# BiaPyX/BiaPy

Measured on AMD Instinct MI355X. Metric: voxels/sec 3D ResUNet 128^3 patch (train: fwd+bwd+AdamW; sub-records: infer, sliding), higher is better.
Workload: dtype f16 forward/activations + bf16 gradients (MFMA f16 / bf16, fp32 accumulate)

## Files before the change

### biapy_amd/_lib.py

```python
from __future__ import annotations

import ctypes as C
import os
from typing import Optional

import torch

_HERE = os.path.dirname(os.path.abspath(__file__))
LIB_PATH = os.environ.get("BPX_LIB_PATH") or os.path.join(_HERE, "libbiapy_amd.so")

F32, BF16, F16, U8, MIX16 = 0, 1, 2, 3, 4
U16 = 5
I32 = 6
ACT = {"none": 0, "linear": 0, "elu": 1, "relu": 2, "silu": 3, "leaky_relu": 4, "gelu": 5, "tanh": 6, "sigmoid": 7, "softplus": 8}
PK_K3, PK_K3_T, PK_K1, PK_DENSE, PK_DENSE_T, PK_CT, PK_CT_T, PK_CT4, PK_CT4_T = range(9)


class AxisGrid(C.Structure):
    _fields_ = [("n", C.c_int32), ("step", C.c_int32), ("last", C.c_int32), ("patch", C.c_int32), ("limit", C.c_int32)]


class Tensor(C.Structure):
    _fields_ = [("ptr", C.c_void_p), ("ld", C.c_int32), ("C", C.c_int32), ("cs", C.c_int64)]


NULL_T = Tensor(None, 0, 0, 0)

_vp, _i, _i64, _f = C.c_void_p, C.c_int, C.c_int64, C.c_float

_SIGS = {
    "bpx_version": ([], C.c_int),
    "bpx_last_error": ([], C.c_char_p),
    "bpx_selftest_layouts": ([_vp, _vp], _i),
    "bpx_debug_set_wgrad_tr": ([_i], _i),
    "bpx_debug_set_conv_ws": ([_i], _i),
    "bpx_debug_set_conv_stamps": ([_vp], _i),
    "bpx_debug_set_tiling_scalar": ([_i], _i),
    "bpx_debug_set_conv_occ": ([_i], _i),
    "bpx_debug_set_conv_zm": ([_i], _i),
    "bpx_debug_conv_zm_launches": ([], _i),
    "bpx_debug_conv_zm_occupancy": ([_i], _i),
    "bpx_crop3d_gather": ([_vp, _i, _i, _i, _i, _i, _i, _i, _i, _i, C.POINTER(AxisGrid), _i64, _i64, _vp, _vp], _i),
    "bpx_merge3d_blend": ([_vp, _i, _i, _i, _i, _i, _i, _i, _i, C.POINTER(AxisGrid), _vp, _vp, _vp, _i, _i, _i, _i, _i, _i, _i,
                           _vp, _vp, _i, _vp, _i, _vp], _i),
    "bpx_packed_weight_elems": ([_i, _i, _i, _i], _i64),
    "bpx_pack_weight": ([_i, _vp, _i, _i, _i, _vp, _vp], _i),
    "bpx_pack_weights_batched": ([_i, _i, _vp, _vp], _i),
    "bpx_adam_step": ([_i, _vp, _vp, C.c_double, C.c_double, C.c_double, C.c_double, C.c_double, _i, _vp], _i),
    "bpx_grad_norm_workspace": ([_i, _vp], _i64),
    "bpx_grad_norm": ([_i, _vp, C.c_double, _vp, _i64, _vp, _vp], _i),
    "bpx_adam_step_dev": ([_i, _vp, _vp, C.c_double, _vp, C.c_double, C.c_double, C.c_double, C.c_double, _i, _vp, _vp], _i),
    "bpx_sgd_step": ([_i, _vp, _vp, C.c_double, _vp, C.c_double, C.c_double, C.c_double, _i, _vp, _vp], _i),
    "bpx_aug_draw": ([_vp, _i, _i, _i, _i, _vp, _vp, _vp], _i),
    "bpx_aug_mean_blocks": ([_i64], _i),
    "bpx_aug_mean": ([_vp, _i, _i64, _vp, _vp, _vp], _i),
    "bpx_aug_apply": ([_vp, _vp, _i, _i, _i, _i, _i, _i, _i, _vp, C.c_uint64, _f, _i, _vp, _vp, _vp], _i),
    "bpx_warp_draw": ([_vp, _i, _i, _i, _vp, _vp, _vp], _i),
    "bpx_warp_apply": ([_vp, _vp, _i, _i, _i, _i, _i, _i, _i, _vp, _i, _f, _vp, _vp, _vp], _i),
    "bpx_patch_draw": ([_vp, _vp, _vp, _vp, _vp, _i64, _i, _vp, _vp, _vp], _i),
    "bpx_patch_gather": ([_vp, _vp, _i, _i, _i, _i, _i, _i, _i, _i, _vp, _i, _i, _f, _vp, _vp, _vp], _i),
    "bpx_label_workspace": ([_i, _i, _i], _i64),
    "bpx_label_u8": ([_vp, _i, _i, _i, _i, _vp, _vp, _vp, _i64, _vp], _i),
    "bpx_label_sizes": ([_vp, _i64, _i, _vp, _vp], _i),
    "bpx_label_filter": ([_vp, _i64, _i, _vp, _i, _i, _vp, _vp], _i),
    "bpx_debug_set_label_tiled": ([_i], _i),
    "bpx_edt_workspace": ([_i, _i, _i, _i], _i64),
    "bpx_edt": ([_vp, _i, _i, _i, _i, _i, C.POINTER(C.c_double), _i, _vp, _vp, _i64, _vp], _i),
    "bpx_watershed_workspace": ([_i, _i, _i], _i64),
    "bpx_watershed": ([_vp, _i, _vp, _vp, _i, _i, _i, _i, _vp, _vp, _vp, _i64, _vp], _i),
    "bpx_overlap_workspace": ([_i64], _i64),
    "bpx_label_overlap": ([_vp, _vp, _i64, _i64, _vp, _vp, _vp, _vp, _i64, _vp], _i),
    "bpx_debug_set_overlap_per_voxel": ([_i], _i),
    "bpx_region_props": ([_vp, _i, _i, _i, _i, _vp, _vp, _vp, _vp], _i),
    "bpx_debug_set_regionprops_local": ([_i], _i),
    "bpx_morph": ([_vp, _i, _i, _i, _i, _i, _i, _i, _i, _i, _vp, _vp], _i),
    "bpx_peaks_workspace": ([_i, _i, _i], _i64),
    "bpx_peak_local_max": ([_vp, _i, _i, _i, _i, _i, _i, _i, C.c_double, _i, _i, _i, _vp, _vp, _i, _vp, _vp, _i64, _vp], _i),
    "bpx_scan_blocks": ([_i64], _i),
    "bpx_select_workspace": ([], _i64),
    "bpx_select_kth_f32": ([_vp, _i64, _i64, _vp, _vp, _vp], _i),
    "bpx_minmax_f32": ([_vp, _i64, _vp, _vp], _i),
    "bpx_moment_f32": ([_vp, _i64, C.c_double, _i, _vp, _vp], _i),
    "bpx_histogram_f32": ([_vp, _i64, _f, _f, _i, _vp, _vp, _vp], _i),
    "bpx_threshold_u8": ([_vp, _i64, _f, _vp, _vp], _i),
    "bpx_clip_affine_f32": ([_vp, _i64, _f, _f, _f, _f, _vp, _vp], _i),
    "bpx_class_argmax": ([_vp, _i64, _i, _i, _vp, _vp], _i),
    "bpx_tta_orient": ([_vp, _i, _i, _i, _i, _vp, _vp, _vp, _vp], _i),
    "bpx_tta_accumulate": ([_vp, _i, _i, _i, _i, _vp, _vp, _i, _i, _i, _vp, _vp], _i),
    "bpx_chan_loss_blocks": ([_i64], _i),
    "bpx_chan_loss_sums": ([_vp, _vp, _i, _i, _i64, C.c_uint, _vp, _vp], _i),
    "bpx_chan_loss_bwd": ([_vp, _vp, _i, _i, _i64, C.c_uint, _vp, _vp, _vp], _i),
    "bpx_gate_mul_fwd": ([_i, _i64, Tensor, Tensor, Tensor, _vp], _i),
    "bpx_gate_mul_bwd": ([_i, _i64, Tensor, Tensor, Tensor, Tensor, _vp, _vp], _i),
    "bpx_seg_loss_blocks": ([_i64], _i),
    "bpx_seg_loss_sums": ([_vp, _vp, _i64, _vp, _vp], _i),
    "bpx_seg_loss_bwd": ([_vp, _vp, _i64, _vp, _vp, _vp], _i),
    "bpx_seg_loss_finish": ([_vp, _i, _i64, _f, _f, _f, _vp, _vp, _vp], _i),
    "bpx_seg_loss_bwd_fused": ([_vp, _vp, _i64, _vp, _vp, _f, _f, _f, _vp, _vp], _i),
    "bpx_softmax_ce_blocks": ([_i64], _i),
    "bpx_softmax_ce_row": ([], _i),
    "bpx_softmax_ce_sums": ([_vp, _vp, _i, _i, _i64, _i, _vp, _vp, _vp], _i),
    "bpx_softmax_ce_finish": ([_vp, _i, _i64, _vp, _vp, _vp], _i),
    "bpx_softmax_ce_bwd": ([_vp, _vp, _i, _i, _i64, _i, _vp, _vp, _vp, _vp, _vp], _i),
    "bpx_dice_blocks": ([_i64], _i),
    "bpx_dice_row": ([], _i),
    "bpx_dice_sums": ([_vp, _vp, _i, _i, _i64, _i, _i, _vp, _i, _vp, _vp], _i),
    "bpx_dice_finish": ([_vp, _i, _i, _i64, _i, _i, C.c_double, C.c_double, C.c_double, _vp, _vp, _vp, _vp], _i),
    "bpx_dice_bwd": ([_vp, _vp, _i, _i, _i64, _i, _i, _i, _vp, _vp, _vp, _vp, _vp], _i),
    "bpx_chan_loss_finish": ([_vp, _i, _i, _i64, _vp, _vp, _vp], _i),
    "bpx_chan_loss_bwd_fused": ([_vp, _vp, _i, _i, _i64, C.c_uint, _vp, _vp, _vp, _vp], _i),
    "bpx_conv3d_fwd": ([_i, _i, _i, _i, _i, Tensor, _vp, _i, _vp, _vp, Tensor, _vp, _vp, Tensor, _vp, _vp], _i),
    "bpx_conv3d_fwd_pool": ([_i, _i, _i, _i, _i, Tensor, _vp, _i, _vp, _vp, Tensor, _vp, _vp, Tensor, _vp, _i, Tensor, _vp, _vp], _i),
    "bpx_conv3d_fwd_pool_supported": ([_i, _i, _i, _i, _i, _i, _i, _i], _i),
    "bpx_conv3d_fwd_shuffle": ([_i, _i, _i, _i, _i, Tensor, _vp, _i, _vp, _vp, _i, Tensor, _vp], _i),
    "bpx_conv3d_stats_tiles": ([_i, _i, _i, _i, _i, _i], _i),
    "bpx_conv3d_dgrad": ([_i, _i, _i, _i, _i, Tensor, _vp, Tensor, _vp, _i, Tensor, _vp, _vp], _i),
    "bpx_conv3d_wgrad": ([_i, _i, _i, _i, _i, Tensor, _vp, _i, Tensor, _i, _vp, _vp, _vp, _i64, _vp], _i),
    "bpx_conv3d_wgrad_db2": ([_i, _i, _i, _i, _i, Tensor, _vp, _i, Tensor, _i, _vp, _vp, _vp, _vp, _i64, _vp], _i),
    "bpx_conv3d_wgrad_workspace": ([_i, _i, _i, _i, _i, _i, _i], _i64),
    "bpx_conv3d_bwd_fused_supported": ([_i, _i, _i, _i, _i, _i, _i], _i),
    "bpx_conv3d_bwd_fused_stats_tiles": ([_i, _i, _i, _i, _i, _i], _i),
    "bpx_conv3d_bwd_fused_workspace": ([_i, _i, _i, _i, _i, _i], _i64),
    "bpx_conv3d_bwd_fused": ([_i, _i, _i, _i, _i, Tensor, _vp, Tensor, _vp, _i, Tensor, _vp, _vp, _vp, _vp, _vp, _i64, _vp], _i),
    "bpx_debug_set_bwd_fused": ([_i], _i),
# ... 261 lines not shown
```

### biapy_amd/csrc/conv3d_zmarch.hip

```cpp
#include "conv3d_shared.h"

using namespace bpxconv;

namespace {

#ifndef BPX_ZM_IMG_EARLY
#define BPX_ZM_IMG_EARLY 1
#endif

#ifndef BPX_ZM_RH
#define BPX_ZM_RH 4
#endif
#ifndef BPX_ZM_SCK_AH
#define BPX_ZM_SCK_AH 2
#endif
#ifndef BPX_ZM_SCK_RH
#define BPX_ZM_SCK_RH 2
#endif
constexpr int zm_occ(int nch, bool sck = false) { return (nch == 1 && !sck) ? 3 : 2; }

template <int NCH, int ACTK, bool F16, bool SCK = false>
__global__ void __launch_bounds__(256, zm_occ(NCH, SCK)) conv3_zm_kernel(const Conv3Params p) {
  using T = typename std::conditional<F16, f16_t, uint16_t>::type;
  constexpr int TZ = 4, TY = 8, TX = 16, MS = 8, KPL = 8, VB = 32, HY = TY + 2, HX = TX + 2;
  constexpr int PLANE_B = HY * HX * VB;
  constexpr int PP = HY * HX * 2;
  constexpr int PL = PP - 256;
  static_assert(2 * PL <= 256, "a plane pair's left-over pieces fit one round");
  constexpr int STEPS = 14, QPAD = 56, HSTR = HX * VB;
  constexpr int RH = NCH != 1 ? MS : SCK ? BPX_ZM_SCK_RH : BPX_ZM_RH;
  constexpr int PLANES = NCH == 1 ? 6 : 2 + 4 * NCH;
  constexpr int RING_B = PLANES * PLANE_B;
  constexpr int WLDS_B = NCH == 1 ? STEPS * 1024 : 0;
  constexpr int RED_B = (NCH == 1 ? 2 : 1) * 4 * 16 * 2 * 4;
  constexpr int TAB_B = NCH * 16 * 8 + 128;
  constexpr int POOL_B = NCH == 1 ? 2 * (MS / 2) * 32 * 8 : 0;
  constexpr int WOFF = RING_B, ROFF = WOFF + WLDS_B, TOFF = ROFF + RED_B, POFF = TOFF + TAB_B;
  __shared__ __attribute__((aligned(16))) unsigned char smem[POFF + POOL_B];
  float* const red = reinterpret_cast<float*>(smem + ROFF);
  float* const tab = reinterpret_cast<float*>(smem + TOFF);

  const int tid = threadIdx.x, lane = tid & 63;
  const int wave = __builtin_amdgcn_readfirstlane(tid >> 6);
  const int j = lane & 15, g = lane >> 4;
  const int D = p.D, H = p.H, W = p.W;
  constexpr int Cout = 16;
  const int cg_off = (g & 1) * 16;
  const bool hi_tap = (g >> 1) != 0;
  const uint32_t hb = (uint32_t)(j * VB + cg_off);

#ifdef BPX_ZM_STAMPS
  long long* stamps = (p.stamps && tid == 0) ? p.stamps + (size_t)blockIdx.x * 16 : nullptr;
  int stamp_i = 0, it = 0;
#define ZM_STAMP() do { if (stamps && it == 4 && stamp_i < 15) stamps[stamp_i++] = (long long)__builtin_readcyclecounter(); } while (0)
#define ZM_STEP_DONE() ++it
#else
#define ZM_STAMP() do { } while (0)
#define ZM_STEP_DONE() do { } while (0)
#endif

  const int sub = tid & 1;
  const int hvA = tid >> 1, hyA = hvA / HX, hxA = hvA - hyA * HX;
  const int selL = tid / PL, idxL = 256 + (tid - selL * PL), hvL = idxL >> 1, hyL = hvL / HX, hxL = hvL - hyL * HX;
  const bool hasL = tid < 2 * PL;
  const uint32_t HWB = (uint32_t)(H * W * p.x_ld) * 2u;
  uint32_t relA = (uint32_t)((hyA * W + hxA) * p.x_ld + sub * KPL) * 2u;
  uint32_t relL = (uint32_t)((hyL * W + hxL) * p.x_ld + sub * KPL) * 2u + (hasL ? (uint32_t)selL * HWB : 0u);
  asm volatile("" : "+v"(relA), "+v"(relL));
  const uint32_t ldsA = (uint32_t)tid * 16u, ldsL = (uint32_t)idxL * 16u;
  const char* __restrict__ xin = reinterpret_cast<const char*>(p.x);
  const char* __restrict__ wp = reinterpret_cast<const char*>(p.wp);
  const uint32_t wlane = (uint32_t)((g * Cout + j) * KPL) * 2u;
  const uint32_t x_csb = (uint32_t)p.x_cs * 2u, sc_csb = (uint32_t)p.sc_cs * 2u;

  const bool rank1 = p.sc != nullptr && p.sc_C == 1;
  float* const ektab = tab + NCH * 16 * 2;
  if (tid < 16) {
    float a = 0.f;
    if (p.bias) a += p.bias[tid];
    if (p.sc && p.bias_sc) a += p.bias_sc[tid];
    ektab[tid] = a;
    ektab[16 + tid] = rank1 ? reinterpret_cast<const float*>(p.wsc)[tid] : 0.f;
  }
  if constexpr (NCH == 1) {
#pragma unroll
    for (int q = tid; q < STEPS * 64; q += 256)
      *reinterpret_cast<u32x4_t*>(smem + WOFF + q * 16) = *reinterpret_cast<const u32x4_t*>(wp + (uint32_t)q * 16u);
  }

  const int tilesZ = p.tilesZ, colsPerSample = p.tilesY * p.tilesX;
  const int xcd = blockIdx.x & 7, slot = blockIdx.x >> 3, spx = gridDim.x >> 3;
  const int T8 = p.tilesPerXcd;
  int L0 = xcd * T8 + (int)(((long long)slot * T8) / spx), L1 = xcd * T8 + (int)(((long long)(slot + 1) * T8) / spx);
  {
    const int cap = min((xcd + 1) * T8, p.totalTiles);
    L1 = min(L1, cap);
  }
  if (L0 >= L1) return;
  int col = L0 / tilesZ, tzi = L0 - col * tilesZ;

  int n = 0, y0 = 0, x0 = 0, tyi = 0, txi = 0;
// ... 586 lines not shown
      for (int k = 0; k < MS / 2; ++k) {
        u32x2_t pk[2];
#pragma unroll
        for (int h = 0; h < 2; ++h) {
          const int ms = 2 * k + h;
          const bool in = okzx && ms < yrem;
          float v[4];
#pragma unroll
          for (int r = 0; r < 4; ++r) {
            const float t = acc[ms][r] + addk[r] + img[ms] * w1k[r];
            v[r] = in ? t : 0.f;
            s1[r] += v[r];
            s2[r] += v[r] * v[r];
          }
          pk[h] = u32x2_t{pk16s<T>(v[0], v[1]), pk16s<T>(v[2], v[3])};
          __builtin_amdgcn_raw_buffer_store_b64(pk[h], rs_y, (int)(in ? yb0 + ms * yrow : 0xFFFFFFFFu), 0, 0);
        }
        if (p.pool != nullptr) {
          const u32x2_t a = pk[0], b = pk[1];
          m[k][0] = fmaxf(lo16<T>(a[0]), lo16<T>(b[0])); m[k][1] = fmaxf(hi16<T>(a[0]), hi16<T>(b[0]));
          m[k][2] = fmaxf(lo16<T>(a[1]), lo16<T>(b[1])); m[k][3] = fmaxf(hi16<T>(a[1]), hi16<T>(b[1]));
#pragma unroll
          for (int r = 0; r < 4; ++r)
            m[k][r] = fmaxf(m[k][r], __builtin_bit_cast(float, __builtin_amdgcn_update_dpp(0, __builtin_bit_cast(int, m[k][r]), 0xB1, 0xF, 0xF, true)));
        }
      }
      if (p.part != nullptr) {
        float* red = reinterpret_cast<float*>(smem + ROFF) + par * 256;
#pragma unroll
        for (int r = 0; r < 4; ++r) {
          const float a = row16_sum(s1[r]), b = row16_sum(s2[r]);
          if (j == 0) *reinterpret_cast<f32x2_t*>(&red[(wave * 16 + g * 4 + r) * 2]) = f32x2_t{a, b};
        }
      }
      if (pool2 && (wave & 1)) {
        u32x2_t* ex = reinterpret_cast<u32x2_t*>(smem + POFF);
#pragma unroll
        for (int k = 0; k < MS / 2; ++k) ex[((wave >> 1) * (MS / 2) + k) * 32 + (lane >> 1)] = u32x2_t{pk16<T>(m[k][0], m[k][1]), pk16<T>(m[k][2], m[k][3])};
      }
    }
    if (pool2) __syncthreads();
    if (p.pool != nullptr) {
      float q1[4] = {0.f, 0.f, 0.f, 0.f}, q2[4] = {0.f, 0.f, 0.f, 0.f};
      if (pool2 && !(wave & 1)) {
        const u32x2_t* ex = reinterpret_cast<const u32x2_t*>(smem + POFF);
#pragma unroll
        for (int k = 0; k < MS / 2; ++k) {
          const u32x2_t o = ex[((wave >> 1) * (MS / 2) + k) * 32 + (lane >> 1)];
          m[k][0] = fmaxf(m[k][0], lo16<T>(o[0])); m[k][1] = fmaxf(m[k][1], hi16<T>(o[0]));
          m[k][2] = fmaxf(m[k][2], lo16<T>(o[1])); m[k][3] = fmaxf(m[k][3], hi16<T>(o[1]));
        }
      }
      if ((p.pool_sz == 1 || !(wave & 1)) && !(j & 1) && z0 + wave < D && x0 + j < W) {
        const int Dp = D / p.pool_sz, Hp = H >> 1, Wp = W >> 1;
        const int pz_ = (z0 + wave) / p.pool_sz, px = (x0 + j) >> 1;
        char* __restrict__ pout = reinterpret_cast<char*>(p.pool);
#pragma unroll
        for (int k = 0; k < MS / 2; ++k) {
          if (y0 + 2 * k < H) {
            const int py = (y0 >> 1) + k;
            *reinterpret_cast<u32x2_t*>(pout + (uint32_t)((((n * Dp + pz_) * Hp + py) * Wp + px) * p.pool_ld + g * 4) * 2u) =
                u32x2_t{pk16<T>(m[k][0], m[k][1]), pk16<T>(m[k][2], m[k][3])};
#pragma unroll
            for (int r = 0; r < 4; ++r) { q1[r] += m[k][r]; q2[r] += m[k][r] * m[k][r]; }
          }
        }
      }
      if (p.pool_part != nullptr) {
        float* red = reinterpret_cast<float*>(smem + ROFF) + par * 256 + 128;
#pragma unroll
        for (int r = 0; r < 4; ++r) {
          const float a = row16_sum(q1[r]), b = row16_sum(q2[r]);
          if (j == 0) *reinterpret_cast<f32x2_t*>(&red[(wave * 16 + g * 4 + r) * 2]) = f32x2_t{a, b};
        }
      }
    }
    __syncthreads();
    ZS_STEP_END()
  }
#undef ZS_STEP_BEGIN
#undef ZS_STEP_END
}

int g_zm_mode = -1;
int g_zm_wgs = 0;
int g_zm_launches = 0;

}

extern "C" int bpx_debug_conv_zm_launches(void) { return g_zm_launches; }
extern "C" int bpx_debug_conv_zm_occupancy(int nch) {
  int n = 0;
  hipError_t e = nch == 0   ? hipOccupancyMaxActiveBlocksPerMultiprocessor(&n, conv3_zs_kernel<1, true>, 512, 0)
                 : nch == 1 ? hipOccupancyMaxActiveBlocksPerMultiprocessor(&n, conv3_zm_kernel<1, 1, true>, 256, 0)
                            : hipOccupancyMaxActiveBlocksPerMultiprocessor(&n, conv3_zm_kernel<3, 1, true>, 256, 0);
  return e == hipSuccess ? n : -1;
}
extern "C" int bpx_debug_set_conv_zm(int mode) {
  g_zm_mode = mode < 0 ? -1 : (mode & 0xFF);
  g_zm_wgs = mode < 0 ? 0 : (mode >> 8);
  return 0;
}

namespace bpxconv {

static int zm_cu_count() {
  static int n = 0;
  if (n == 0) {
    int dev = 0, v = 0;
    n = (hipGetDevice(&dev) == hipSuccess && hipDeviceGetAttribute(&v, hipDeviceAttributeMultiprocessorCount, dev) == hipSuccess && v > 0) ? v : 256;
  }
  return n;
}

int launch_conv3_zm(const Conv3Params& p0, const TileCfg& c, hipStream_t s) {
  int mode = g_zm_mode, wgs = g_zm_wgs;
  if (mode < 0) {
    static const char* e = getenv("BPX_CONV_ZM");
    const int v = e ? atoi(e) : 1;
    mode = v & 0xFF; wgs = v >> 8;
  }
  const bool no_zs = (mode & 4) != 0;
  mode &= 3;
  if (mode == 0) return 1;
  if (!(c.tz == 4 && c.ty == 8 && c.tx == 16 && c.ns == 1) || p0.Cout != 16 || p0.ps > 1) return 1;
  if (!(p0.Cin == 16 || p0.Cin == 48)) return 1;
  if (p0.pool != nullptr && p0.Cin != 16) return 1;
  {
    static const char* e = getenv("BPX_CONV_ZM_MASK");
    static const int mask = e ? atoi(e) : 7;
    const int kind = p0.Cin == 48 ? 4 : (p0.sc != nullptr && p0.sc_C >= 16) ? 2 : 1;
    if (!(mask & kind)) return 1;
  }
  Conv3Params p = p0;
  p.tilesZ = cdiv(p.D, c.tz);
  p.tilesY = cdiv(p.H, c.ty);
  p.tilesX = cdiv(p.W, c.tx);
  p.tilesPerSample = p.tilesZ * p.tilesY * p.tilesX;
  p.totalTiles = p.N * p.tilesPerSample;
  p.tilesPerXcd = cdiv(p.totalTiles, 8);
  p.stamps = g_conv_stamps;
  p.dbg = 0;
  const int nch = p.Cin / 16;
  const bool sck = p.sc != nullptr && p.sc_C >= 16;
  {
    static const char* e = getenv("BPX_CONV_ZS");
    static const int zs = e ? atoi(e) : 1;
    if (zs && !no_zs && nch == 1 && !sck) {
      int gz = std::max(8, (zm_cu_count() * 2) & ~7);
      if (wgs > 0) gz = std::max(8, std::min(gz, wgs & ~7));
      gz = std::min(gz, 8 * p.tilesPerXcd);
      if (mode == 1 && (p.totalTiles < 4 * gz || p.tilesZ < 4)) return 1;
      const bool elu_ = p.act == BPX_ACT_ELU;
      ++g_zm_launches;
      dim3 gridz((unsigned)gz, 1);
      if (p.f16) { if (elu_) conv3_zs_kernel<1, true><<<gridz, 512, 0, s>>>(p); else conv3_zs_kernel<0, true><<<gridz, 512, 0, s>>>(p); }
      else { if (elu_) conv3_zs_kernel<1, false><<<gridz, 512, 0, s>>>(p); else conv3_zs_kernel<0, false><<<gridz, 512, 0, s>>>(p); }
      return 0;
    }
  }
  if (sck && (p.sc_C > 48 || nch != 1)) return 1;
  const int occ = zm_occ(nch, sck);
  int gx = std::max(8, (zm_cu_count() * occ) & ~7);
  if (wgs > 0) gx = std::max(8, std::min(gx, wgs & ~7));
  gx = std::min(gx, 8 * p.tilesPerXcd);
  if (mode == 1 && (p.totalTiles < 4 * gx || p.tilesZ < 4)) return 1;
  const bool elu = p.act == BPX_ACT_ELU;
  dim3 grid((unsigned)gx, 1);
#define Z(NCH, SCK)                                                                    \
  if (nch == NCH && sck == SCK) {                                                      \
    ++g_zm_launches;                                                                   \
    if (p.f16) {                                                                       \
      if (elu) conv3_zm_kernel<NCH, 1, true, SCK><<<grid, 256, 0, s>>>(p);             \
      else conv3_zm_kernel<NCH, 0, true, SCK><<<grid, 256, 0, s>>>(p);                 \
    } else {                                                                           \
      if (elu) conv3_zm_kernel<NCH, 1, false, SCK><<<grid, 256, 0, s>>>(p);            \
      else conv3_zm_kernel<NCH, 0, false, SCK><<<grid, 256, 0, s>>>(p);                \
    }                                                                                  \
    return 0;                                                                          \
  }
  Z(1, false) Z(1, true) Z(3, false)
#undef Z
  return 1;
}

}
```

### include/biapy_amd.h

```cpp
#ifndef BIAPY_AMD_H
#define BIAPY_AMD_H

#include <stdint.h>

#ifdef __cplusplus
extern "C" {
#endif

typedef void* bpx_stream_t;

enum bpx_dtype { BPX_F32 = 0, BPX_BF16 = 1, BPX_F16 = 2, BPX_U8 = 3,
                 BPX_MIX16 = 4,
                 BPX_U16 = 5,
                 BPX_I32 = 6 };
enum bpx_act { BPX_ACT_NONE = 0, BPX_ACT_ELU = 1, BPX_ACT_RELU = 2, BPX_ACT_SILU = 3, BPX_ACT_LEAKY_RELU = 4, BPX_ACT_GELU = 5, BPX_ACT_TANH = 6,
               BPX_ACT_SIGMOID = 7, BPX_ACT_SOFTPLUS = 8, BPX_ACT_LAST = 8 };
enum bpx_pad_mode { BPX_PAD_REFLECT = 0, BPX_PAD_ZEROS = 1 };

int bpx_version(void);
const char* bpx_last_error(void);
int bpx_selftest_layouts(float* out_d , bpx_stream_t stream);
int bpx_debug_set_wgrad_tr(int use_tr);
int bpx_debug_set_conv_stamps(void* stamps_d);
int bpx_debug_set_conv_ws(int on);
int bpx_debug_set_conv_occ(int wg_per_cu);
int bpx_debug_set_conv_zm(int mode);
int bpx_debug_conv_zm_launches(void);
int bpx_debug_conv_zm_occupancy(int nch);
int bpx_debug_set_c1_persist(int wgs);
int bpx_debug_set_convt_k1(int on);
int bpx_debug_set_pw_stream(int on);
int bpx_debug_set_wgrad_k1(int on);
int bpx_debug_set_wgrad_cap(int percent);
int bpx_debug_set_tile_order(int bits);
int bpx_debug_set_tiling_scalar(int on);

typedef struct bpx_axis_grid {
  int32_t n, step, last, patch, limit;
} bpx_axis_grid;

int bpx_crop3d_gather(const void* vol_d, int elem_size, int Z, int Y, int X, int C,
                      int pad_z, int pad_y, int pad_x, int pad_mode,
                      const bpx_axis_grid* grid_zyx ,
                      int64_t c_begin, int64_t c_count, void* out_d, bpx_stream_t stream);

int bpx_merge3d_blend(const void* patches_d, int dtype, int Pz, int Py, int Px, int C,
                      int pad_z, int pad_y, int pad_x,
                      const bpx_axis_grid* grid_zyx ,
                      const float* wz_d, const float* wy_d, const float* wx_d,
                      int Z, int Y, int X, int z_lo, int z_hi, int zrow_lo, int zrow_hi,
                      float* acc_d, float* wacc_d, int write_partial,
                      void* out_d, int out_dtype, bpx_stream_t stream);

int bpx_gather3d_tables(const void* vol_d, int elem_size, int Z, int Y, int X, int C, const int* tables_d, int n, int Pz, int Py, int Px,
                        void* out_d, bpx_stream_t stream);
int bpx_scatter3d_tables(const void* in_d, int elem_size, const int* tables_d, int n, int Pz, int Py, int Px, void* vol_d, int Z, int Y,
                         int X, int C, bpx_stream_t stream);
int bpx_scatter3d_regions(const float* pred_d, int n, int Pz, int Py, int Px, int C, const int* regions_d, float* out_d, int Z, int Y,
                          int X, bpx_stream_t stream);


typedef struct bpx_norm_rec {
  float mean, rstd, scale, shift;
} bpx_norm_rec;

typedef struct bpx_tensor {
  void* ptr;
  int32_t ld;
  int32_t C;
  int64_t cs;
} bpx_tensor;

enum bpx_pack_mode { BPX_PK_K3 = 0, BPX_PK_K3_T = 1, BPX_PK_K1 = 2, BPX_PK_DENSE = 3, BPX_PK_DENSE_T = 4, BPX_PK_CT = 5, BPX_PK_CT_T = 6,
                     BPX_PK_CT4 = 7, BPX_PK_CT4_T = 8 };
int64_t bpx_packed_weight_elems(int mode, int Cin, int Cout, int dtype);
int bpx_pack_weight(int mode, const float* w_d, int Cin, int Cout, int dtype, void* packed_d, bpx_stream_t stream);
typedef struct bpx_pack_job {
  const float* w_d;
  void* packed_d;
  int32_t mode, Cin, Cout, reserved;
} bpx_pack_job;
int bpx_pack_weights_batched(int dtype, int count, const bpx_pack_job* jobs, bpx_stream_t stream);

typedef struct bpx_adam_tensor {
  float* p; const float* g; float* m; float* v;
  float* step;
  int64_t numel;
} bpx_adam_tensor;
int bpx_adam_step(int count, const bpx_adam_tensor* tensors, const float* lr_d, double lr, double beta1, double beta2, double eps,
                  double weight_decay, int decoupled, bpx_stream_t stream);

int64_t bpx_grad_norm_workspace(int count, const bpx_adam_tensor* tensors);
int bpx_grad_norm(int count, const bpx_adam_tensor* tensors, double max_norm, void* workspace_d, int64_t workspace_bytes, float* out_d,
                  bpx_stream_t stream);
int bpx_adam_step_dev(int count, const bpx_adam_tensor* tensors, const float* lr_d, double lr, const double* beta1_d, double beta1, double beta2,
                      double eps, double weight_decay, int decoupled, const float* gscale_d, bpx_stream_t stream);
int bpx_sgd_step(int count, const bpx_adam_tensor* tensors, const float* lr_d, double lr, const double* momentum_d, double momentum,
                 double dampening, double weight_decay, int nesterov, const float* gscale_d, bpx_stream_t stream);

int bpx_conv3d_fwd(int dtype, int N, int D, int H, int W, bpx_tensor x, const bpx_norm_rec* in_norm_d, int act,
                   const void* w_packed_d, const float* bias_d, bpx_tensor sc, const void* w_sc_packed_d,
                   const float* bias_sc_d, bpx_tensor y, float* stats_part_d, bpx_stream_t stream);
int bpx_conv3d_stats_tiles(int dtype, int N, int D, int H, int W, int Cout);
int bpx_conv3d_fwd_pool(int dtype, int N, int D, int H, int W, bpx_tensor x, const bpx_norm_rec* in_norm_d, int act,
                        const void* w_packed_d, const float* bias_d, bpx_tensor sc, const void* w_sc_packed_d,
                        const float* bias_sc_d, bpx_tensor y, float* stats_part_d, int pool_sz, bpx_tensor pooled,
                        float* pool_stats_part_d, bpx_stream_t stream);
int bpx_conv3d_fwd_pool_supported(int dtype, int N, int D, int H, int W, int x_ld, int y_ld, int Cout);
int bpx_conv3d_fwd_shuffle(int dtype, int N, int D, int H, int W, bpx_tensor x, const bpx_norm_rec* in_norm_d, int act, const void* w_packed_d,
                           const float* bias_d, int s, bpx_tensor y, bpx_stream_t stream);

// ... 322 lines not shown
```

Measured before the change: 1.075 billion.

## Add warp-specialized producer/consumer conv3d kernel for 48-channel inputs

Adds a new 768-thread conv3d kernel for Cin=48 layers without a wide shortcut. It splits each workgroup into 256 MFMA consumer threads and 512 producer threads that prefetch halo planes, apply the fused input normalization and activation, and write them into double-buffered LDS. It also keeps the weights for all three channel chunks in LDS. The aim is to overlap global loads with compute on these layers, which previously ran the NCH=3 zm kernel. The costs are more LDS per workgroup, a grid capped at one workgroup per CU, and per-chunk block barriers.

New measurement: 1.077 billion (median of 6 runs). No clear change (+0.2%).

```diff
diff --git a/biapy_amd/_lib.py b/biapy_amd/_lib.py
--- a/biapy_amd/_lib.py
+++ b/biapy_amd/_lib.py
@@ -40,6 +40,7 @@
     "bpx_debug_set_conv_zm": ([_i], _i),
     "bpx_debug_conv_zm_launches": ([], _i),
     "bpx_debug_conv_zm_occupancy": ([_i], _i),
+    "bpx_debug_conv_zs_launches": ([_i], _i),
     "bpx_crop3d_gather": ([_vp, _i, _i, _i, _i, _i, _i, _i, _i, _i, C.POINTER(AxisGrid), _i64, _i64, _vp, _vp], _i),
     "bpx_merge3d_blend": ([_vp, _i, _i, _i, _i, _i, _i, _i, _i, C.POINTER(AxisGrid), _vp, _vp, _vp, _i, _i, _i, _i, _i, _i, _i,
                            _vp, _vp, _i, _vp, _i, _vp], _i),
diff --git a/biapy_amd/csrc/conv3d_zmarch.hip b/biapy_amd/csrc/conv3d_zmarch.hip
--- a/biapy_amd/csrc/conv3d_zmarch.hip
+++ b/biapy_amd/csrc/conv3d_zmarch.hip
@@ -17,6 +17,10 @@
 #ifndef BPX_ZM_SCK_RH
 #define BPX_ZM_SCK_RH 2
 #endif
+#ifndef BPX_ZS3_PD
+#define BPX_ZS3_PD 2
+#endif
+constexpr int ZS3_THREADS = 768;
 constexpr int zm_occ(int nch, bool sck = false) { return (nch == 1 && !sck) ? 3 : 2; }
 
 template <int NCH, int ACTK, bool F16, bool SCK = false>
@@ -769,16 +773,329 @@
 #undef ZS_STEP_END
 }
 
+
+template <int ACTK, bool F16>
+__global__ void __launch_bounds__(ZS3_THREADS, 3) conv3_zs3_kernel(const Conv3Params p) {
+  using T = typename std::conditional<F16, f16_t, uint16_t>::type;
+  constexpr int NCH = 3, TZ = 4, TY = 8, TX = 16, MS = 8, KPL = 8, VB = 32, HY = TY + 2, HX = TX + 2;
+  constexpr int PLANE_B = HY * HX * VB, PP = HY * HX * 2;
+  constexpr int STEPS = 14, HSTR = HX * VB;
+  constexpr int PRIV_B = 4 * PLANE_B;
+  constexpr int WREG = NCH * PRIV_B;
+  constexpr int RING_B = WREG + 4 * PLANE_B;
+  constexpr int WOFF = RING_B, WCH_B = STEPS * 1024;
+  constexpr int ROFF = WOFF + NCH * WCH_B, RED_B = 4 * 16 * 2 * 4;
+  constexpr int TOFF = ROFF + RED_B;
+  constexpr int NT = ZS3_THREADS, NP = NT - 256;
+  constexpr int NOFF = TOFF + 128, NTAB_B = NCH * 16 * 8;
+  __shared__ __attribute__((aligned(16))) unsigned char smem[NOFF + (NP / 64) * NTAB_B];
+  float* const red = reinterpret_cast<float*>(smem + ROFF);
+  float* const ektab = reinterpret_cast<float*>(smem + TOFF);
+  static_assert(NP < 2 * PP && 2 * NP >= 2 * PP && NP >= PP, "a plane pair is one piece per producer thread and a second one for the first 2 PP - NP threads, all of them in the pair's second plane");
+
+  const int tid = threadIdx.x, lane = tid & 63;
+  const bool producer = tid >= 256;
+  const int ptid = producer ? tid - 256 : tid;
+  const int wave = __builtin_amdgcn_readfirstlane(ptid >> 6);
+  const int j = lane & 15, g = lane >> 4;
+  const int D = p.D, H = p.H, W = p.W;
+  constexpr int Cout = 16;
+
+  const bool rank1 = p.sc != nullptr && p.sc_C == 1;
+  if (tid < 16) {
+    float a = 0.f;
+    if (p.bias) a += p.bias[tid];
+    if (p.sc && p.bias_sc) a += p.bias_sc[tid];
+    ektab[tid] = a;
+    ektab[16 + tid] = rank1 ? reinterpret_cast<const float*>(p.wsc)[tid] : 0.f;
+  }
+  for (int q = tid; q < NCH * STEPS * 64; q += NT)
+    *reinterpret_cast<u32x4_t*>(smem + WOFF + q * 16) = *reinterpret_cast<const u32x4_t*>(reinterpret_cast<const char*>(p.wp) + (uint32_t)q * 16u);
+
+  const int tilesZ = p.tilesZ, colsPerSample = p.tilesY * p.tilesX;
+  const int xcd = blockIdx.x & 7, slot = blockIdx.x >> 3, spx = gridDim.x >> 3;
+  const int T8 = p.tilesPerXcd;
+  int L0 = xcd * T8 + (int)(((long long)slot * T8) / spx), L1 = xcd * T8 + (int)(((long long)(slot + 1) * T8) / spx);
+  {
+    const int cap = min((xcd + 1) * T8, p.totalTiles);
+    L1 = min(L1, cap);
+  }
+  if (L0 >= L1) return;
+
+#ifdef BPX_ZM_STAMPS
+  long long* stamps = (p.stamps && ptid == 0) ? p.stamps + (size_t)blockIdx.x * 16 + (producer ? 8 : 0) : nullptr;
+  int stamp_i = 0, it = 0;
+#define ZS3_STAMP() do { if (stamps && it == 4 && stamp_i < 8) stamps[stamp_i++] = (long long)__builtin_readcyclecounter(); } while (0)
+#define ZS3_STEP_DONE() ++it
+#else
+#define ZS3_STAMP() do { } while (0)
+#define ZS3_STEP_DONE() do { } while (0)
+#endif
+
+  int off = 0, wr = 0;
+  auto plane = [&](int q, int c) -> uint32_t {
+    if (q == 2 || q == 3) return (uint32_t)(WREG + (wr * 2 + (q - 2)) * PLANE_B);
+    const int par = q < 2 ? off : (off ^ 1);
+    return (uint32_t)(c * PRIV_B + (par * 2 + (q & 1)) * PLANE_B);
+  };
+  auto decode = [&](int L, int& n, int& tzi, int& tyi, int& txi) {
+    const int col = L / tilesZ;
+    tzi = L - col * tilesZ;
+    n = col / colsPerSample;
+    const int r = col - n * colsPerSample;
+    tyi = r / p.tilesX; txi = r - tyi * p.tilesX;
+  };
+
+  if (producer) {
+    const int sub = ptid & 1;
+    const int selA = ptid >= PP ? 1 : 0, idxA = ptid - selA * PP, hvA = idxA >> 1, hyA = hvA / HX, hxA = hvA - hyA * HX;
+    const bool hasB = ptid < 2 * PP - NP;
+    const int idxB = hasB ? NP - PP + ptid : 0, hvB = idxB >> 1, hyB = hvB / HX, hxB = hvB - hyB * HX;
+    const uint32_t HWB = (uint32_t)(H * W * p.x_ld) * 2u;
+    uint32_t relA = (uint32_t)((hyA * W + hxA) * p.x_ld + sub * KPL) * 2u + (uint32_t)selA * HWB;
+    uint32_t relB = (uint32_t)((hyB * W + hxB) * p.x_ld + sub * KPL) * 2u + HWB;
+    asm volatile("" : "+v"(relA), "+v"(relB));
+    const uint32_t ldsA = (uint32_t)idxA * 16u, ldsB = (uint32_t)idxB * 16u;
+    const char* __restrict__ xin = reinterpret_cast<const char*>(p.x);
+    const uint32_t x_csb = (uint32_t)p.x_cs * 2u;
+    const bool has_norm = p.in_norm != nullptr;
+
+    uint32_t colb = 0;
+    bool okA = false, okB = false, q_new = true;
+    int q_z0 = 0, q_n = 0, q_row = 0;
+    auto request_step = [&](int L) {
+      int tzi, tyi, txi;
+      decode(L, q_n, tzi, tyi, txi);
+      const int y0 = tyi * TY, x0 = txi * TX;
+      colb = (uint32_t)(((q_n * D) * H + (y0 - 1)) * W + (x0 - 1)) * (uint32_t)p.x_ld * 2u;
+      okA = (unsigned)(y0 - 1 + hyA) < (unsigned)H && (unsigned)(x0 - 1 + hxA) < (unsigned)W;
+      okB = hasB && (unsigned)(y0 - 1 + hyB) < (unsigned)H && (unsigned)(x0 - 1 + hxB) < (unsigned)W;
+      q_z0 = tzi * TZ;
+      q_new = L == L0 || tzi == 0;
+      q_row = q_n * p.tilesPerSample + (tzi * p.tilesY + tyi) * p.tilesX + txi;
+    };
+    auto load_pair = [&](u32x4_t* v, uint32_t& mask, int bit, int z, int c) {
+      const uint32_t cb = colb + (uint32_t)c * x_csb + (uint32_t)z * HWB;
+      const bool oa = okA && (unsigned)(z + selA) < (unsigned)D, ob = okB && (unsigned)(z + 1) < (unsigned)D;
+      v[0] = *reinterpret_cast<const u32x4_t*>(xin + (oa ? cb + relA : 0u));
+      v[1] = *reinterpret_cast<const u32x4_t*>(xin + (ob ? cb + relB : 0u));
+      mask |= (oa ? 1u << bit : 0u) | (ob ? 2u << bit : 0u);
+    };
+    auto request_stage = [&](u32x4_t* v, uint32_t& mask, int c) {
+      mask = 0;
+      if (q_new) load_pair(v + 4, mask, 4, q_z0 - 1, c);
+      load_pair(v, mask, 0, q_z0 + 1, c);
+      load_pair(v + 2, mask, 2, q_z0 + 3, c);
+    };
+    auto store_pair = [&](const u32x4_t* v, uint32_t mask, int bit, uint32_t s0, uint32_t s1, const float* psc, const float* psh) {
+#pragma unroll
+      for (int k = 0; k < 2; ++k) {
+        if (k == 1 && !hasB) break;
+        u32x4_t t = v[k];
+        const bool in = (mask >> (bit + k)) & 1u;
+        if (!in) t = u32x4_t{0u, 0u, 0u, 0u};
+        if (has_norm && in) {
+#pragma unroll
+          for (int i = 0; i < 4; ++i) {
+            float a = fmaf(psc[2 * i], lo16<T>(t[i]), psh[2 * i]), b = fmaf(psc[2 * i + 1], hi16<T>(t[i]), psh[2 * i + 1]);
+            act_pair<ACTK>(a, b, p.act);
+            t[i] = pk16<T>(a, b);
+          }
+        }
+        const uint32_t dst = k == 0 ? (selA ? s1 : s0) + ldsA : s1 + ldsB;
+        *reinterpret_cast<u32x4_t*>(smem + dst) = t;
+      }
+    };
+    auto store_row = [&](int row) {
+      if (row < 0 || p.part == nullptr || ptid >= 32) return;
+      const int ch = ptid >> 1, k = ptid & 1;
+      const float a = red[(0 * 16 + ch) * 2 + k] + red[(1 * 16 + ch) * 2 + k] + red[(2 * 16 + ch) * 2 + k] + red[(3 * 16 + ch) * 2 + k];
+      p.part[((size_t)row * 2 + k) * Cout + ch] = a;
+    };
+
+    float* const wtab = reinterpret_cast<float*>(smem + NOFF + __builtin_amdgcn_readfirstlane(ptid >> 6) * NTAB_B);
+    int tab_n = -1;
+    constexpr int PD = BPX_ZS3_PD, RD = PD - 1;
+    static_assert(RD >= 1 && RD <= NCH, "a request reaches into the next step at most");
+    u32x4_t buf[PD][6];
+    uint32_t mask[PD];
+    request_step(L0);
+#pragma unroll
+    for (int k = 0; k < RD; ++k) request_stage(buf[k], mask[k], k);
+    bool s_new = q_new;
+    int s_n = q_n, s_row = q_row, prev_row = -1;
+    for (int L = L0; L < L1; ++L) {
+#pragma unroll
+      for (int c = 0; c < NCH; ++c) {
+        if (c == 0) ZS3_STAMP();
+        mask[RD] = 0;
+        if (c + RD < NCH) request_stage(buf[RD], mask[RD], c + RD);
+        else if (L + 1 < L1) {
+          if (c + RD == NCH) request_step(L + 1);
+          request_stage(buf[RD], mask[RD], c + RD - NCH);
+        }
+        if (c == 0) ZS3_STAMP();
+        if (c == 0 && has_norm && s_n != tab_n) {
+          tab_n = s_n;
+          if (lane < NCH * 16) *reinterpret_cast<f32x2_t*>(wtab + lane * 2) = *reinterpret_cast<const f32x2_t*>(&p.in_norm[(size_t)s_n * p.Cin + lane].scale);
+          asm volatile("" ::: "memory");
+        }
+        float psc[KPL], psh[KPL];
+        if (has_norm) {
+          const f32x4_t* tp = reinterpret_cast<const f32x4_t*>(wtab + (c * 16 + sub * KPL) * 2);
+#pragma unroll
+          for (int i = 0; i < 4; ++i) {
+            const f32x4_t q = tp[i];
+            psc[2 * i] = q[0]; psh[2 * i] = q[1]; psc[2 * i + 1] = q[2]; psh[2 * i + 1] = q[3];
+          }
+        }
+        if (c == 1) store_row(prev_row);
+        if (s_new) store_pair(buf[0] + 4, mask[0], 4, plane(0, c), plane(1, c), psc, psh);
+        store_pair(buf[0], mask[0], 0, plane(2, c), plane(3, c), psc, psh);
+        store_pair(buf[0] + 2, mask[0], 2, plane(4, c), plane(5, c), psc, psh);
+        ZS3_STAMP();
+        __syncthreads();
+        ZS3_STAMP();
+        wr ^= 1;
+#pragma unroll
+        for (int d = 0; d < RD; ++d) {
+#pragma unroll
+          for (int k = 0; k < 6; ++k) buf[d][k] = buf[d + 1][k];
+          mask[d] = mask[d + 1];
+        }
+      }
+      ZS3_STEP_DONE();
+      off ^= 1;
+      prev_row = s_row;
+      s_new = q_new; s_n = q_n; s_row = q_row;
+    }
+    __syncthreads();
+    store_row(prev_row);
+    return;
+  }
+
+  const int cg_off = (g & 1) * 16;
+  const bool hi_tap = (g >> 1) != 0;
+  const uint32_t hb = (uint32_t)(j * VB + cg_off);
+  const uint32_t hb0 = hb + (hi_tap ? VB : 0), hb1 = hb + (hi_tap ? HX * VB : 0);
+  const uint32_t wl = WOFF + (uint32_t)lane * 16u;
+  const __amdgpu_buffer_rsrc_t rs_y = __builtin_amdgcn_make_buffer_rsrc(p.y, 0, (int)0xFFFFFFF0u, 0x00020000);
+  const uint32_t yrow = (uint32_t)(W * p.y_ld) * 2u;
+
+  for (int L = L0; L < L1; ++L) {
+    int n, tzi, tyi, txi;
+    decode(L, n, tzi, tyi, txi);
+    const int z0 = tzi * TZ, y0 = tyi * TY, x0 = txi * TX;
+    const bool full = z0 + TZ <= D && y0 + TY <= H && x0 + TX <= W;
+    const int vox0 = ((n * D + z0 + wave) * H + y0) * W + x0 + j;
+    const bool okzx = full || (z0 + wave < D && x0 + j < W);
+    const int yrem = full ? (1 << 20) : H - y0;
+    ZS3_STAMP();
+    f32x4_t acc[MS];
+#pragma unroll
+    for (int ms = 0; ms < MS; ++ms) acc[ms] = f32x4_t{0.f, 0.f, 0.f, 0.f};
+
+#pragma unroll
+    for (int c = 0; c < NCH; ++c) {
+      __syncthreads();
+      ZS3_STAMP();
+      const uint32_t pz[3] = {plane(wave, c), plane(wave + 1, c), plane(wave + 2, c)};
+      const uint32_t wc = wl + c * WCH_B;
+      constexpr int HB = MS / 2;
+      u32x4_t fr[2][HB + 2], wf[2][3];
+      auto read_batch = [&](int b, u32x4_t* f, u32x4_t* w) {
+        const int grp = b >> 1, h = (b & 1) * HB;
+        if (grp < 3) {
+          const uint32_t b0 = pz[grp] + hb0;
+          if (h == 0) {
+#pragma unroll
+            for (int dy = 0; dy < 3; ++dy) w[dy] = *reinterpret_cast<const u32x4_t*>(smem + wc + (3 * grp + dy) * 1024);
+          }
+#pragma unroll
+          for (int r = 0; r < HB + 2; ++r) f[r] = *reinterpret_cast<const u32x4_t*>(smem + b0 + (h + r) * HSTR);
+        } else {
+          const int s = grp + 6;
+          const uint32_t base = s < 12 ? pz[s < 12 ? s - 9 : 0] + hb1 : s == 12 ? (hi_tap ? pz[1] : pz[0]) + hb : pz[2] + hb;
+          const int imm = s < 12 ? 2 * VB : (2 * HX + 2) * VB;
+          if (h == 0) w[0] = *reinterpret_cast<const u32x4_t*>(smem + wc + s * 1024);
+#pragma unroll
+          for (int ms = 0; ms < HB; ++ms) f[ms] = *reinterpret_cast<const u32x4_t*>(smem + base + (h + ms) * HSTR + imm);
+        }
+      };
+      read_batch(0, fr[0], wf[0]);
+#pragma unroll
+      for (int b = 0; b < 16; ++b) {
+        if (b + 1 < 16) read_batch(b + 1, fr[(b + 1) & 1], wf[((b + 1) >> 1) & 1]);
+        __builtin_amdgcn_sched_barrier(0);
+        const u32x4_t* f = fr[b & 1];
+        const u32x4_t* w = wf[(b >> 1) & 1];
+        const int h = (b & 1) * HB;
+        if (b < 6) {
+#pragma unroll
+          for (int dy = 0; dy < 3; ++dy)
+#pragma unroll
+            for (int ms = 0; ms < HB; ++ms) acc[h + ms] = mfma_step<T>(w[dy], f[ms + dy], acc[h + ms]);
+        } else {
+#pragma unroll
+          for (int ms = 0; ms < HB; ++ms) acc[h + ms] = mfma_step<T>(w[0], f[ms], acc[h + ms]);
+        }
+        __builtin_amdgcn_sched_barrier(0);
+      }
+      ZS3_STAMP();
+      wr ^= 1;
+    }
+
+    const uint32_t yb0 = (uint32_t)(vox0 * p.y_ld + g * 4) * 2u;
+    const f32x4_t addk = *reinterpret_cast<const f32x4_t*>(ektab + g * 4), w1k = *reinterpret_cast<const f32x4_t*>(ektab + 16 + g * 4);
+    float img[MS];
+#pragma unroll
+    for (int ms = 0; ms < MS; ++ms)
+      img[ms] = rank1 ? *reinterpret_cast<const float*>(reinterpret_cast<const char*>(p.sc) + ((okzx && ms < yrem) ? (uint32_t)(vox0 + ms * W) * 4u : 0u)) : 0.f;
+    __builtin_amdgcn_s_waitcnt(0x0070);
+    float s1[4] = {0.f, 0.f, 0.f, 0.f}, s2[4] = {0.f, 0.f, 0.f, 0.f};
+#pragma unroll
+    for (int ms = 0; ms < MS; ++ms) {
+      const bool in = okzx && ms < yrem;
+      float v[4];
+#pragma unroll
+      for (int r = 0; r < 4; ++r) {
+        const float t = acc[ms][r] + addk[r] + img[ms] * w1k[r];
+        v[r] = in ? t : 0.f;
+        s1[r] += v[r];
+        s2[r] += v[r] * v[r];
+      }
+      const u32x2_t pk = u32x2_t{pk16s<T>(v[0], v[1]), pk16s<T>(v[2], v[3])};
+      __builtin_amdgcn_raw_buffer_store_b64(pk, rs_y, (int)(in ? yb0 + ms * yrow : 0xFFFFFFFFu), 0, 0);
+    }
+    if (p.part != nullptr) {
+#pragma unroll
+      for (int r = 0; r < 4; ++r) {
+        const float a = row16_sum(s1[r]), b = row16_sum(s2[r]);
+        if (j == 0) *reinterpret_cast<f32x2_t*>(&red[(wave * 16 + g * 4 + r) * 2]) = f32x2_t{a, b};
+      }
+    }
+    ZS3_STAMP();
+    ZS3_STEP_DONE();
+    off ^= 1;
+  }
+  __syncthreads();
+#undef ZS3_STAMP
+#undef ZS3_STEP_DONE
+}
+
 int g_zm_mode = -1;
 int g_zm_wgs = 0;
 int g_zm_launches = 0;
+int g_zs_launches[2] = {0, 0};
 
 }
 
 extern "C" int bpx_debug_conv_zm_launches(void) { return g_zm_launches; }
+extern "C" int bpx_debug_conv_zs_launches(int nch) { return nch == 1 ? g_zs_launches[0] : nch == 3 ? g_zs_launches[1] : -1; }
 extern "C" int bpx_debug_conv_zm_occupancy(int nch) {
   int n = 0;
   hipError_t e = nch == 0   ? hipOccupancyMaxActiveBlocksPerMultiprocessor(&n, conv3_zs_kernel<1, true>, 512, 0)
+                 : nch == -3 ? hipOccupancyMaxActiveBlocksPerMultiprocessor(&n, conv3_zs3_kernel<1, true>, ZS3_THREADS, 0)
                  : nch == 1 ? hipOccupancyMaxActiveBlocksPerMultiprocessor(&n, conv3_zm_kernel<1, 1, true>, 256, 0)
                             : hipOccupancyMaxActiveBlocksPerMultiprocessor(&n, conv3_zm_kernel<3, 1, true>, 256, 0);
   return e == hipSuccess ? n : -1;
@@ -840,9 +1157,23 @@
       if (mode == 1 && (p.totalTiles < 4 * gz || p.tilesZ < 4)) return 1;
       const bool elu_ = p.act == BPX_ACT_ELU;
       ++g_zm_launches;
+      ++g_zs_launches[0];
       dim3 gridz((unsigned)gz, 1);
       if (p.f16) { if (elu_) conv3_zs_kernel<1, true><<<gridz, 512, 0, s>>>(p); else conv3_zs_kernel<0, true><<<gridz, 512, 0, s>>>(p); }
       else { if (elu_) conv3_zs_kernel<1, false><<<gridz, 512, 0, s>>>(p); else conv3_zs_kernel<0, false><<<gridz, 512, 0, s>>>(p); }
+      return 0;
+    }
+    if (zs && !no_zs && nch == 3 && !sck) {
+      int gz = std::max(8, zm_cu_count() & ~7);
+      if (wgs > 0) gz = std::max(8, std::min(gz, wgs & ~7));
+      gz = std::min(gz, 8 * p.tilesPerXcd);
+      if (mode == 1 && (p.totalTiles < 4 * gz || p.tilesZ < 4)) return 1;
+      const bool elu_ = p.act == BPX_ACT_ELU;
+      ++g_zm_launches;
+      ++g_zs_launches[1];
+      dim3 gridz((unsigned)gz, 1);
+      if (p.f16) { if (elu_) conv3_zs3_kernel<1, true><<<gridz, ZS3_THREADS, 0, s>>>(p); else conv3_zs3_kernel<0, true><<<gridz, ZS3_THREADS, 0, s>>>(p); }
+      else { if (elu_) conv3_zs3_kernel<1, false><<<gridz, ZS3_THREADS, 0, s>>>(p); else conv3_zs3_kernel<0, false><<<gridz, ZS3_THREADS, 0, s>>>(p); }
       return 0;
     }
   }
diff --git a/include/biapy_amd.h b/include/biapy_amd.h
--- a/include/biapy_amd.h
+++ b/include/biapy_amd.h
@@ -27,6 +27,7 @@
 int bpx_debug_set_conv_zm(int mode);
 int bpx_debug_conv_zm_launches(void);
 int bpx_debug_conv_zm_occupancy(int nch);
+int bpx_debug_conv_zs_launches(int nch);
 int bpx_debug_set_c1_persist(int wgs);
 int bpx_debug_set_convt_k1(int on);
 int bpx_debug_set_pw_stream(int on);
```
